# ksahlin/NGSpeciesID

Hardware: AMD Instinct MI355X
Metric: reads/sec end-to-end (cluster + spoa consensus + racon x3), 750 bp ONT (higher is better)
Workload: dtype u8 / int16 / int32 DP, 64-bit bit-vectors (f64 thresholds)

## Files before the change

### ngspeciesid_amd/csrc/k_ed_align.hip

```cpp
#include "ngsid_internal.h"
#include <algorithm>

typedef unsigned long long u64;
#define LDSP __attribute__((address_space(3)))

#define CLIP_RUN 15
template <int BMAX, bool WIN, bool CLIP = false, bool REC = false>
__global__ __launch_bounds__(64) __attribute__((amdgpu_waves_per_eu(2, 4)))
void k_ed_align(AlignJob J, ngsid_v4u* __restrict__ tb, u64 tb_per_wave , uint32_t mstride, uint32_t* __restrict__ work_ctr, int32_t* __restrict__ dist_out,
                int8_t* __restrict__ hcar ,
                int bandK , uint32_t* __restrict__ fail_list, uint32_t* __restrict__ fail_count,
                uint32_t* __restrict__ rec , uint32_t rec_stride)
{
    extern __shared__ __attribute__((aligned(16))) unsigned char smem[];
    const int lane = threadIdx.x;
    LDSP u64* planes = (LDSP u64*)smem;
    ngsid_v4u* mytb = tb + (u64)blockIdx.x * tb_per_wave;
    int8_t* myh = hcar + (u64)blockIdx.x * mstride * 64;
    const u64 npairs1 = J.npairs_dev ? (u64)*J.npairs_dev : J.npairs;
    const u64 npairs = npairs1 + (J.npairs_dev2 ? (u64)*J.npairs_dev2 : 0);
    const u64 nbundles = (npairs + 63) / 64;
    for (;;) {
        uint32_t kq = 0; if (lane == 0) kq = atomicAdd(work_ctr, 1u);
        kq = (uint32_t)__builtin_amdgcn_readfirstlane((int)kq);
        if (kq >= nbundles) break;
        const u64 pk = (u64)kq * 64 + lane;
        const bool have = pk < npairs;
        const u64 p = have ? (J.pair_list ? (pk < npairs1 ? (u64)J.pair_list[pk] : (u64)J.pair_list2[pk - npairs1]) : pk) : 0;
        const uint8_t* q = nullptr; const uint8_t* t = nullptr; int n = 0, m = 0;
        if (have) { const uint32_t qi = J.qidx[p], ti = J.tidx[p]; q = J.qseq + J.qoff[qi]; n = (int)(J.qoff[qi + 1] - J.qoff[qi]); t = J.tseq + J.toff[ti]; m = (int)(J.toff[ti + 1] - J.toff[ti]); }
        int nmax = n, mmax = m;
#pragma unroll
        for (int d = 32; d >= 1; d >>= 1) { nmax = max(nmax, __shfl_xor(nmax, d)); mmax = max(mmax, __shfl_xor(mmax, d)); }
        nmax = __builtin_amdgcn_readfirstlane(nmax); mmax = __builtin_amdgcn_readfirstlane(mmax);
        const int B = (nmax + 63) >> 6;
        const int bl = n > 0 ? (n - 1) >> 6 : 0, lastbit = n > 0 ? (n - 1) & 63 : 0;
        int score = n, best = n, bestj = 0;
        const bool band = bandK > 0 && (WIN || B <= BMAX);
        int dmin = 0, lbprev = -1, sb = 0;
        if (band) {
            dmin = have ? n - m : 0x3fffffff;
#pragma unroll
            for (int d = 32; d >= 1; d >>= 1) dmin = min(dmin, __shfl_xor(dmin, d));
            dmin = __builtin_amdgcn_readfirstlane(dmin);
        }
        if (WIN) {
            const int span = ((2 * bandK + 2 - (dmin < 0 ? dmin : 0)) >> 6) + 2;
            if (span > BMAX) {
                if (have) fail_list[atomicAdd(fail_count, 1u)] = (uint32_t)p;
                continue;
            }
        }
        int fbw = 0;
        for (int g0 = 0; g0 < B; g0 += (WIN ? B : BMAX)) {
            const int Bg = min(BMAX, B - g0);
            auto build_planes = [&](int blk, int slot) {
                u64 lo = 0, hi = 0, ok = 0;
                const int base = blk * 64;
                for (int r = 0; r < 64; ++r) {
                    const int i = base + r;
                    const int c = i < n ? ngsid_bcode(q[i]) : 4;
                    lo |= (u64)(c & 1) << r; hi |= (u64)((c >> 1) & 1) << r; ok |= (u64)(c < 4) << r;
                }
                planes[(slot * 3 + 0) * 64 + lane] = lo; planes[(slot * 3 + 1) * 64 + lane] = hi; planes[(slot * 3 + 2) * 64 + lane] = ok;
            };
            for (int b = 0; b < Bg; ++b) build_planes(g0 + b, b);
            u64 Pv[BMAX], Mv[BMAX];
#pragma unroll
            for (int b = 0; b < BMAX; ++b) { Pv[b] = ~0ull; Mv[b] = 0ull; }
            const bool more = !WIN && g0 + BMAX < B;
            u64 TPlo = 0, TPhi = 0, TPok = 0;
            for (int j = 0; j < mmax; ++j) {
                const int jb = j & 63;
                if (jb == 0) {
                    u64 lo = 0, hi = 0, ok = 0;
#pragma unroll 16
                    for (int c = 0; c < 64; ++c) {
                        const int jc = j + c;
                        const int cd = jc < m ? ngsid_bcode(t[jc]) : 4;
                        lo |= (u64)(cd & 1) << c; hi |= (u64)((cd >> 1) & 1) << c; ok |= (u64)(cd < 4) << c;
                    }
                    TPlo = lo; TPhi = hi; TPok = ok;
                }
                const u64 Tlo = 0ull - ((TPlo >> jb) & 1ull), Thi = 0ull - ((TPhi >> jb) & 1ull), Tok = 0ull - ((TPok >> jb) & 1ull);
                int fb = 0, lb = Bg - 1;
                if (band) {
                    const int lo_row = j + dmin - bandK - 1;
                    fb = lo_row > 0 ? (lo_row >> 6) : 0; lb = min(B - 1, (j + 1 + bandK) >> 6);
                    if (lb > lbprev) {
                        if (n > 0 && bl > lbprev && bl <= lb) score = sb + 64 * (bl - 1 - lbprev) + lastbit + 1;
                        sb += 64 * (lb - lbprev);
                    }
                }
                if (WIN) {
                    while (fb > fbw) {
#pragma unroll
                        for (int b = 0; b + 1 < BMAX; ++b) { Pv[b] = Pv[b + 1]; Mv[b] = Mv[b + 1]; }
                        Pv[BMAX - 1] = ~0ull; Mv[BMAX - 1] = 0ull;
                        ++fbw;
                        const int nb = fbw + BMAX - 1;
                        if (nb < B) build_planes(nb, nb % BMAX);
                    }
                }
                unsigned hp, hm;
                if (g0) { const int h0 = (int)myh[(u64)j * 64 + lane]; hp = h0 > 0; hm = h0 < 0; }
                else { hp = fb > 0 ? 1u : 0u; hm = 0u; }
                ngsid_v4u* col = mytb + ((u64)j * 64 + lane);
                const int slot0 = WIN ? fbw % BMAX : 0;
                const bool inm = j < m;
#pragma unroll
                for (int b = 0; b < BMAX; ++b) {
                    const int blk = WIN ? fbw + b : g0 + b;
                    if (WIN ? blk <= lb : (b >= fb && b <= lb)) {
                        const int ps = WIN ? (slot0 + b >= BMAX ? slot0 + b - BMAX : slot0 + b) : b;
                        const u64 lo = planes[(ps * 3 + 0) * 64 + lane], hi = planes[(ps * 3 + 1) * 64 + lane], ok = planes[(ps * 3 + 2) * 64 + lane];
                        const u64 Eq = ~((lo ^ Tlo) | (hi ^ Thi)) & ok & Tok;
                        const u64 pv = Pv[b], mv = Mv[b];
                        const u64 Xv = Eq | mv;
                        const u64 Eqh = Eq | (u64)hm;
                        const u64 Xh = (((Eqh & pv) + pv) ^ pv) | Eqh;
                        u64 Ph = mv | ~(Xh | pv), Mh = pv & Xh;
                        const u64 diag = Eq | (Ph & ~(pv | mv)) | (~(Ph | Mh) & pv);
                        if (blk == bl && inm) {
                            score += (int)((Ph >> lastbit) & 1) - (int)((Mh >> lastbit) & 1);
                            if (score < best) { best = score; bestj = j + 1; }
                        }
                        const unsigned php = (unsigned)(Ph >> 63), phm = (unsigned)(Mh >> 63);
                        Ph = (Ph << 1) | (u64)hp; Mh = (Mh << 1) | (u64)hm;
                        const u64 npv = Mh | ~(Xv | Ph);
                        Pv[b] = npv; Mv[b] = Ph & Xv;
                        ngsid_v4u w; w.x = (unsigned)diag; w.y = (unsigned)(diag >> 32); w.z = (unsigned)npv; w.w = (unsigned)(npv >> 32);
#if defined(ED_EXP_STORE_EVERY)
                        if ((j % ED_EXP_STORE_EVERY) == 0)
#endif
                        col[(u64)(WIN ? b : blk) * mstride * 64] = w;
                        hp = php; hm = phm;
                    }
                }
                if (more) myh[(u64)j * 64 + lane] = (int8_t)((int)hp - (int)hm);
                if (band) { sb += (int)hp - (int)hm; lbprev = lb; }
            }
            if (more) { asm volatile("s_waitcnt vmcnt(0)" ::: "memory"); __builtin_amdgcn_wave_barrier(); }
        }
        asm volatile("s_waitcnt vmcnt(0)" ::: "memory");
        __builtin_amdgcn_wave_barrier();
        bool ok = true;
        if (band && have && best > bandK) { ok = false; fail_list[atomicAdd(fail_count, 1u)] = (uint32_t)p; }
        int i = ok ? n : 0, j = bestj;
        int q_end = -1, t_end = -1, q_beg = -1, t_beg = -1;
        int32_t* bpp = (J.bp && have) ? J.bp + p * (u64)J.bp_windows * 4 : nullptr;
        if (bpp) for (int x = 0; x < J.bp_windows * 4; ++x) bpp[x] = -1;
        const int W = J.window > 0 ? J.window : 0x7fffffff;
        int cw = -1, w_qf = 0, w_ql = 0, w_tf = 0, w_tl = 0;
        int c_run = 0, c_x0q = -1, c_x0t = -1; bool c_started = false;
        uint32_t r_acc = 0; int r_w = -1;
        uint32_t* myrec = (REC && have) ? rec + p * (u64)rec_stride : nullptr;
        auto rec_put = [&](int ti, uint32_t nib) { const int w_ = ti >> 3; if (w_ != r_w) { if (r_w >= 0) myrec[r_w] = r_acc; r_acc = 0; r_w = w_; } r_acc |= nib << ((ti & 7) * 4); };
        int wsn = j > 0 ? (j - 1) / W : 0, ws = wsn * W;
        auto tb_blk = [&](int ii, int col0) { int tb_ = (ii - 1) >> 6; if (WIN) { const int lo_row = col0 + dmin - bandK - 1; tb_ -= lo_row > 0 ? (lo_row >> 6) : 0; } return tb_; };
        auto tb_load = [&](int tb_, int col0) { return __builtin_nontemporal_load(mytb + (((u64)tb_ * mstride + (u64)col0) * 64 + lane)); };
        int jj = i > 0 ? j : 0;
#if defined(ED_EXP_NO_TB)
        jj = 0;
#endif
#pragma unroll
        for (int d = 32; d >= 1; d >>= 1) jj = max(jj, __shfl_xor(jj, d));
        jj = __builtin_amdgcn_readfirstlane(jj);
        ngsid_v4u wn; wn.x = wn.y = wn.z = wn.w = 0; int wn_blk = -0x7fffffff;
        if (i > 0 && j == jj && jj >= 1) { wn_blk = tb_blk(i, jj - 1); wn = tb_load(wn_blk, jj - 1); }
        for (; jj >= 1; --jj) {
            if (!__ballot(i > 0 && j > 0)) break;
            const bool on = i > 0 && j == jj;
            ngsid_v4u w = wn; int wb = wn_blk;
            wn_blk = -0x7fffffff;
            if (jj >= 2) {
                int gi = 0;
                if (on && i > 1) gi = i - 1;
                else if (i > 0 && j == jj - 1) gi = i;
                if (gi > 0) { wn_blk = tb_blk(gi, jj - 2); wn = tb_load(wn_blk, jj - 2); }
            }
            if (on) {
                { const int nb = tb_blk(i, jj - 1); if (nb != wb) { w = tb_load(nb, jj - 1); wb = nb; } }
                uint32_t r_ins = 0;
                for (;;) {
                    const int bit = (i - 1) & 63;
                    const u64 dv = ((u64)w.y << 32) | w.x, uv = ((u64)w.w << 32) | w.z;
                    const bool diag = (dv >> bit) & 1, up = (uv >> bit) & 1;
                    if (diag) {
                        const int qi0 = i - 1, ti0 = j - 1;
                        auto record = [&](int qi, int ti) {
                            if (q_end < 0) { q_end = qi; t_end = ti; }
                            q_beg = qi; t_beg = ti;
                            if (bpp) {
                                while (ti < ws) { ws -= W; --wsn; }
                                const int wn_ = wsn;
                                if (wn_ != cw) { if (cw >= 0 && cw < J.bp_windows) { bpp[cw * 4 + 0] = w_qf; bpp[cw * 4 + 1] = w_ql; bpp[cw * 4 + 2] = w_tf; bpp[cw * 4 + 3] = w_tl; } cw = wn_; w_ql = qi; w_tl = ti; }
                                w_qf = qi; w_tf = ti;
                            }
                        };
                        if constexpr (CLIP) {
                            const uint8_t cq = q[qi0] & 0xDF, ct = t[ti0] & 0xDF;
                            const bool eq = cq == ct && (cq == 'A' || cq == 'C' || cq == 'G' || cq == 'T');
                            c_run = eq ? c_run + 1 : 0;
                            if (!c_started) {
                                if (c_run >= CLIP_RUN) {
                                    c_started = true;
                                    for (int d = CLIP_RUN - 1; d >= 0; --d) record(qi0 + d, ti0 + d);
                                    c_x0q = qi0; c_x0t = ti0;
                                }
                            } else {
                                record(qi0, ti0);
                                if (c_run >= CLIP_RUN) { c_x0q = qi0; c_x0t = ti0; }
                            }
                        } else record(qi0, ti0);
                        if constexpr (REC) {
                            const int cq = ngsid_bcode(q[qi0]), ct = ngsid_bcode(t[ti0]);
                            rec_put(ti0, (cq < 4 ? (cq == ct ? (uint32_t)NGSID_REC_EQ : (uint32_t)NGSID_REC_SUB + cq) : (uint32_t)NGSID_REC_OTHER) | r_ins);
                        }
                        --i; --j; break;
                    }
                    if constexpr (CLIP) c_run = 0;
                    if (!up) { if constexpr (REC) rec_put(j - 1, (uint32_t)NGSID_REC_DEL | r_ins); --j; break; }
                    --i;
                    if constexpr (REC) r_ins = NGSID_REC_INS;
                    if (i == 0) break;
                    { const int nb = tb_blk(i, jj - 1); if (nb != wb) { w = tb_load(nb, jj - 1); wb = nb; } }
                }
            }
        }
        i = 0;
        if constexpr (REC) { if (r_w >= 0) myrec[r_w] = r_acc; }
        if (bpp && ok && cw >= 0 && cw < J.bp_windows) { bpp[cw * 4 + 0] = w_qf; bpp[cw * 4 + 1] = w_ql; bpp[cw * 4 + 2] = w_tf; bpp[cw * 4 + 3] = w_tl; }
        if constexpr (CLIP) {
            if (have && ok && c_started) {
                q_beg = c_x0q; t_beg = c_x0t;
                if (bpp) { const int w0 = c_x0t / W; for (int x = 0; x < w0 && x < J.bp_windows; ++x) { bpp[x * 4 + 0] = -1; bpp[x * 4 + 1] = -1; bpp[x * 4 + 2] = -1; bpp[x * 4 + 3] = -1; }
                           if (w0 < J.bp_windows) { bpp[w0 * 4 + 0] = c_x0q; bpp[w0 * 4 + 2] = c_x0t; } }
            }
        }
        if (have && ok) {
            if (dist_out) dist_out[p] = best;
            if (J.span) { J.span[p * 4 + 0] = q_beg; J.span[p * 4 + 1] = q_end; J.span[p * 4 + 2] = t_beg; J.span[p * 4 + 3] = t_end; }
        }
        __builtin_amdgcn_wave_barrier();
    }
}

static int32_t ed_reserve(ngsid_ctx* ctx, u64& want, u64 per_wave)
{
    for (;;) {
        if (ctx->ed_tb.n >= want * per_wave) return NGSID_OK;
        hipError_t e = ctx->ed_tb.reserve(want * per_wave);
        if (e == hipSuccess) return NGSID_OK;
        (void)hipGetLastError();
        if (e != hipErrorOutOfMemory || want <= 64) HIPCHK(ctx, e);
        want = std::max<u64>(64, want / 2);
    }
}

struct EdRec { uint32_t* p = nullptr; uint32_t stride = 0; };
template <int BMAX, bool WIN = false, bool CLIP = false, bool REC = false>
static int32_t launch_ed(ngsid_ctx* ctx, const AlignJob& job, uint32_t max_qlen, uint32_t max_tlen, int32_t* dist_out, uint32_t ctr_slot = 14, int bandK = 0, uint32_t fail_slot = 15, uint32_t* fail_list = nullptr, EdRec rec = EdRec())
{
    const u64 nbundles = (job.npairs + 63) / 64;
    const uint32_t mstride = (max_tlen + 63u) & ~63u;
    const u64 nblocks = WIN ? (u64)BMAX : std::max<u64>(1, ((u64)max_qlen + 63) / 64);
    const u64 per_wave = nblocks * mstride * 64;
    const size_t lds = (size_t)BMAX * 3 * 64 * 8 + (size_t)ngsid_opt(ctx, "ed_lds_pad_kb", 0) * 1024;
    int occ = 0;
    HIPCHK(ctx, hipOccupancyMaxActiveBlocksPerMultiprocessor(&occ, k_ed_align<BMAX, WIN, CLIP, REC>, 64, lds));
    if (occ < 1) occ = 1;
    u64 want = std::min<u64>(nbundles, (u64)occ * ctx->n_cu);
    const u64 by_mem = std::max<u64>(1, std::min<size_t>((size_t)24 << 30, ctx->scratch_budget) / (per_wave * 16));
    want = std::max<u64>(1, std::min(want, by_mem));
    { int32_t rr = ed_reserve(ctx, want, per_wave); if (rr) return rr; }
    if (ctx->ed_h.n < want * (u64)mstride * 64) HIPCHK(ctx, ctx->ed_h.reserve(want * (u64)mstride * 64));
    if (ctx->aln_ctr.n < 16) HIPCHK(ctx, ctx->aln_ctr.alloc(16));
    HIPCHK(ctx, hipMemsetAsync(ctx->aln_ctr.p + ctr_slot, 0, sizeof(uint32_t), ctx->stream));
    { ProfScope ps_(ctx, REC ? "k_ed_align_rec" : "k_ed_align"); hipLaunchKernelGGL((k_ed_align<BMAX, WIN, CLIP, REC>), dim3((unsigned)want), dim3(64), lds, ctx->stream, job, ctx->ed_tb.p, per_wave, mstride, ctx->aln_ctr.p + ctr_slot, dist_out, ctx->ed_h.p,
                                                            bandK, fail_list ? fail_list : ctx->ed_fail.p, ctx->aln_ctr.p + fail_slot, rec.p, rec.stride); }
    HIPCHK(ctx, hipGetLastError());
    return NGSID_OK;
}

template <bool REC>
static int32_t launch_ed_fallback(ngsid_ctx* ctx, const AlignJob& job, uint32_t max_qlen, uint32_t max_tlen, int32_t* dist_out, int retryK, EdRec rec)
{
    AlignJob j = job; j.pair_list = ctx->ed_fail.p; j.npairs_dev = ctx->aln_ctr.p + 15; j.pair_list2 = nullptr; j.npairs_dev2 = nullptr;
    if (retryK > 0) {
        HIPCHK(ctx, ctx->ed_fail2.reserve(job.npairs));
        int32_t rc = launch_ed<8, true, false, REC>(ctx, j, max_qlen, max_tlen, dist_out, 6, retryK, 7, ctx->ed_fail2.p, rec);
        if (rc) return rc;
        j.pair_list = ctx->ed_fail2.p; j.npairs_dev = ctx->aln_ctr.p + 7;
    }
    return launch_ed<16, false, false, REC>(ctx, j, max_qlen, max_tlen, dist_out, 13, 0, 15, nullptr, rec);
}

template <bool REC>
static int32_t ed_align_route(ngsid_ctx* ctx, const AlignJob& job, uint32_t max_qlen, uint32_t max_tlen, int32_t* dist_out, EdRec rec)
{
    if (job.npairs == 0) return NGSID_OK;
    if (max_qlen > NGSID_MAX_CONSENSUS_LEN || max_tlen > NGSID_MAX_CONSENSUS_LEN) NGSID_FAIL(ctx, NGSID_ERR_TOO_LONG, "sequence longer than %d in the edit-distance aligner", NGSID_MAX_CONSENSUS_LEN);
    if (job.clip) return launch_ed<16, false, true, REC>(ctx, job, max_qlen, max_tlen, dist_out, 14, 0, 15, nullptr, rec);
    int bandK = 64 + (int)(max_qlen / 32);
    const bool band_set = ngsid_opt(ctx, "ed_band", -1) >= 0;
    if (band_set) bandK = (int)ngsid_opt(ctx, "ed_band", -1);
    const bool win = max_qlen > 1024 && bandK > 0;
    bool win16 = false;
    if (win) {
        if (bandK > 150 && !band_set) { win16 = true; bandK = std::min(64 + (int)(max_qlen / 16), 400); }
        else if (bandK > 150) { win16 = true; bandK = std::min(bandK, 400); }
    }
    if (ctx->aln_ctr.n < 16) HIPCHK(ctx, ctx->aln_ctr.alloc(16));
    if (bandK > 0) HIPCHK(ctx, ctx->ed_fail.reserve(job.npairs));
    if (job.npairs >= 4096 && max_qlen > 256 && !job.pair_list && !ngsid_opt(ctx, "align_noclass", 0)) {
        int32_t rc = ngsid_partition_pairs(ctx, job); if (rc) return rc;
        const u64 n = job.npairs;
        auto cls = [&](int c, uint32_t bound) { AlignJob j = job; j.pair_list = ctx->aln_cls.p + (size_t)c * n; j.npairs_dev = ctx->aln_ctr.p + 8 + c; (void)bound; return j; };
        {
            const uint32_t mstride = (max_tlen + 63u) & ~63u; const u64 nblocks = std::max<u64>(1, ((u64)max_qlen + 63) / 64); const u64 per_wave = nblocks * mstride * 64;
            const u64 want = std::max<u64>(1, std::min<u64>((u64)8 * ctx->n_cu, std::max<u64>(1, std::min<size_t>((size_t)24 << 30, ctx->scratch_budget) / (per_wave * 16))));
            u64 w2 = want; { int32_t rr = ed_reserve(ctx, w2, per_wave); if (rr) return rr; }
            if (ctx->ed_h.n < w2 * (u64)mstride * 64) HIPCHK(ctx, ctx->ed_h.reserve(w2 * (u64)mstride * 64));
        }
        if ((rc = launch_ed<4, false, false, REC>(ctx, cls(0, 256), std::min<uint32_t>(max_qlen, 256), max_tlen, dist_out, 1, bandK, 15, nullptr, rec))) return rc;
        if (max_qlen > 256 && (rc = launch_ed<8, false, false, REC>(ctx, cls(1, 512), std::min<uint32_t>(max_qlen, 512), max_tlen, dist_out, 2, bandK, 15, nullptr, rec))) return rc;
        const bool win_all = ngsid_opt(ctx, "ed_win_all", 1) != 0;
        const bool win2 = win_all && bandK > 0 && bandK <= 150;
        if (max_qlen > 512) {
            AlignJob j2 = cls(2, 768);
            if (win2 && max_qlen > 768) { j2.pair_list2 = ctx->aln_cls.p + (size_t)3 * n; j2.npairs_dev2 = ctx->aln_ctr.p + 8 + 3; }
            const bool win6 = win2 && bandK <= 100 && ngsid_opt(ctx, "ed_win6", 1) != 0;
            if ((rc = win6 ? launch_ed<6, true, false, REC>(ctx, j2, std::min<uint32_t>(max_qlen, 896), max_tlen, dist_out, 3, bandK, 15, nullptr, rec)
                    : win2 ? launch_ed<8, true, false, REC>(ctx, j2, std::min<uint32_t>(max_qlen, 896), max_tlen, dist_out, 3, bandK, 15, nullptr, rec)
                           : launch_ed<12, false, false, REC>(ctx, j2, std::min<uint32_t>(max_qlen, 768), max_tlen, dist_out, 3, bandK, 15, nullptr, rec))) return rc;
        }
        if (max_qlen > 768 && !win2 && (rc = launch_ed<16, false, false, REC>(ctx, cls(3, 896), std::min<uint32_t>(max_qlen, 896), max_tlen, dist_out, 4, bandK, 15, nullptr, rec))) return rc;
        if (max_qlen > 896 && (rc = win16 ? launch_ed<16, true, false, REC>(ctx, cls(4, 0), max_qlen, max_tlen, dist_out, 5, bandK, 15, nullptr, rec) : win ? launch_ed<8, true, false, REC>(ctx, cls(4, 0), max_qlen, max_tlen, dist_out, 5, bandK, 15, nullptr, rec) : launch_ed<16, false, false, REC>(ctx, cls(4, 0), max_qlen, max_tlen, dist_out, 5, bandK, 15, nullptr, rec))) return rc;
        return bandK > 0 ? launch_ed_fallback<REC>(ctx, job, max_qlen, max_tlen, dist_out, win2 ? 180 : 0, rec) : NGSID_OK;
    }
    if (bandK > 0) HIPCHK(ctx, hipMemsetAsync(ctx->aln_ctr.p + 15, 0, sizeof(uint32_t), ctx->stream));
    int32_t rc;
    if (max_qlen <= 256) rc = launch_ed<4, false, false, REC>(ctx, job, max_qlen, max_tlen, dist_out, 14, bandK, 15, nullptr, rec);
    else if (max_qlen <= 512) rc = launch_ed<8, false, false, REC>(ctx, job, max_qlen, max_tlen, dist_out, 14, bandK, 15, nullptr, rec);
    else if (max_qlen <= 768) rc = launch_ed<12, false, false, REC>(ctx, job, max_qlen, max_tlen, dist_out, 14, bandK, 15, nullptr, rec);
    else if (win16) rc = launch_ed<16, true, false, REC>(ctx, job, max_qlen, max_tlen, dist_out, 14, bandK, 15, nullptr, rec);
    else if (win) rc = launch_ed<8, true, false, REC>(ctx, job, max_qlen, max_tlen, dist_out, 14, bandK, 15, nullptr, rec);
    else rc = launch_ed<16, false, false, REC>(ctx, job, max_qlen, max_tlen, dist_out, 14, bandK, 15, nullptr, rec);
    if (rc || bandK <= 0) return rc;
    return launch_ed_fallback<REC>(ctx, job, max_qlen, max_tlen, dist_out, 0, rec);
}

int32_t ngsid_launch_ed_align(ngsid_ctx* ctx, const AlignJob& job, uint32_t max_qlen, uint32_t max_tlen, int32_t* dist_out)
{
    return ed_align_route<false>(ctx, job, max_qlen, max_tlen, dist_out, EdRec());
}

int32_t ngsid_launch_ed_align_rec(ngsid_ctx* ctx, const AlignJob& job, uint32_t max_qlen, uint32_t max_tlen, uint32_t* rec, uint32_t stride)
{
    if (!rec || !job.span || (uint64_t)stride * 8 < max_tlen) NGSID_FAIL(ctx, NGSID_ERR_ARG, "internal: path matrix of the edit-distance aligner missing or too narrow");
    EdRec r; r.p = rec; r.stride = stride;
    return ed_align_route<true>(ctx, job, max_qlen, max_tlen, nullptr, r);
}
```

Baseline: 1.462 million.

## Store band-relative shifted traceback words to cut per-column traceback writes

In the windowed banded Myers kernel, traceback diag/vertical bit-vectors are now re-aligned to the band's lower row with a funnel shift (alignbit) across adjacent blocks. This lets each column store only the minimal number of 64-bit words covering the band instead of all BMAX blocks. The traceback reader computes bit offsets relative to the band base. This cuts global-memory traceback write traffic in exchange for extra shift ALU work and more complex indexing logic.

```diff
diff --git a/ngspeciesid_amd/csrc/k_ed_align.hip b/ngspeciesid_amd/csrc/k_ed_align.hip
--- a/ngspeciesid_amd/csrc/k_ed_align.hip
+++ b/ngspeciesid_amd/csrc/k_ed_align.hip
@@ -5,6 +5,12 @@
 #define LDSP __attribute__((address_space(3)))
 
 #define CLIP_RUN 15
+__device__ __forceinline__ u64 ed_funnel(u64 lo, u64 hi, int sh)
+{
+    const bool up = sh >= 32;
+    const unsigned d0 = up ? (unsigned)(lo >> 32) : (unsigned)lo, d1 = up ? (unsigned)hi : (unsigned)(lo >> 32), d2 = up ? (unsigned)(hi >> 32) : (unsigned)hi;
+    return ((u64)__builtin_amdgcn_alignbit(d2, d1, (unsigned)sh & 31u) << 32) | (u64)__builtin_amdgcn_alignbit(d1, d0, (unsigned)sh & 31u);
+}
 template <int BMAX, bool WIN, bool CLIP = false, bool REC = false>
 __global__ __launch_bounds__(64) __attribute__((amdgpu_waves_per_eu(2, 4)))
 void k_ed_align(AlignJob J, ngsid_v4u* __restrict__ tb, u64 tb_per_wave , uint32_t mstride, uint32_t* __restrict__ work_ctr, int32_t* __restrict__ dist_out,
@@ -44,12 +50,15 @@
             for (int d = 32; d >= 1; d >>= 1) dmin = min(dmin, __shfl_xor(dmin, d));
             dmin = __builtin_amdgcn_readfirstlane(dmin);
         }
+        int relw = 0;
         if (WIN) {
             const int span = ((2 * bandK + 2 - (dmin < 0 ? dmin : 0)) >> 6) + 2;
             if (span > BMAX) {
                 if (have) fail_list[atomicAdd(fail_count, 1u)] = (uint32_t)p;
                 continue;
             }
+            const int nw = (2 * bandK + 3 - (dmin < 0 ? dmin : 0) + 63) >> 6;
+            if (band && nw < min(span, B)) relw = nw;
         }
         int fbw = 0;
         for (int g0 = 0; g0 < B; g0 += (WIN ? B : BMAX)) {
@@ -83,10 +92,11 @@
                     TPlo = lo; TPhi = hi; TPok = ok;
                 }
                 const u64 Tlo = 0ull - ((TPlo >> jb) & 1ull), Thi = 0ull - ((TPhi >> jb) & 1ull), Tok = 0ull - ((TPok >> jb) & 1ull);
-                int fb = 0, lb = Bg - 1;
+                int fb = 0, lb = Bg - 1, rsh = 0;
                 if (band) {
                     const int lo_row = j + dmin - bandK - 1;
                     fb = lo_row > 0 ? (lo_row >> 6) : 0; lb = min(B - 1, (j + 1 + bandK) >> 6);
+                    if (WIN && lo_row > 0) rsh = lo_row & 63;
                     if (lb > lbprev) {
                         if (n > 0 && bl > lbprev && bl <= lb) score = sb + 64 * (bl - 1 - lbprev) + lastbit + 1;
                         sb += 64 * (lb - lbprev);
@@ -108,9 +118,11 @@
                 ngsid_v4u* col = mytb + ((u64)j * 64 + lane);
                 const int slot0 = WIN ? fbw % BMAX : 0;
                 const bool inm = j < m;
+                u64 pdiag = 0, pnpv = 0;
 #pragma unroll
                 for (int b = 0; b < BMAX; ++b) {
                     const int blk = WIN ? fbw + b : g0 + b;
+                    u64 cdiag = 0, cnpv = 0;
                     if (WIN ? blk <= lb : (b >= fb && b <= lb)) {
                         const int ps = WIN ? (slot0 + b >= BMAX ? slot0 + b - BMAX : slot0 + b) : b;
                         const u64 lo = planes[(ps * 3 + 0) * 64 + lane], hi = planes[(ps * 3 + 1) * 64 + lane], ok = planes[(ps * 3 + 2) * 64 + lane];
@@ -130,11 +142,25 @@
                         const u64 npv = Mh | ~(Xv | Ph);
                         Pv[b] = npv; Mv[b] = Ph & Xv;
                         ngsid_v4u w; w.x = (unsigned)diag; w.y = (unsigned)(diag >> 32); w.z = (unsigned)npv; w.w = (unsigned)(npv >> 32);
+                        if (!WIN || !relw) {
 #if defined(ED_EXP_STORE_EVERY)
-                        if ((j % ED_EXP_STORE_EVERY) == 0)
+                            if ((j % ED_EXP_STORE_EVERY) == 0)
 #endif
-                        col[(u64)(WIN ? b : blk) * mstride * 64] = w;
+                            col[(u64)(WIN ? b : blk) * mstride * 64] = w;
+                        }
+                        cdiag = diag; cnpv = npv;
                         hp = php; hm = phm;
+                    }
+                    if (WIN) {
+                        if (relw && b >= 1 && b <= relw && blk - 1 <= lb) {
+                            const u64 rd = ed_funnel(pdiag, cdiag, rsh), rn = ed_funnel(pnpv, cnpv, rsh);
+                            ngsid_v4u w; w.x = (unsigned)rd; w.y = (unsigned)(rd >> 32); w.z = (unsigned)rn; w.w = (unsigned)(rn >> 32);
+#if defined(ED_EXP_STORE_EVERY)
+                            if ((j % ED_EXP_STORE_EVERY) == 0)
+#endif
+                            col[(u64)(b - 1) * mstride * 64] = w;
+                        }
+                        pdiag = cdiag; pnpv = cnpv;
                     }
                 }
                 if (more) myh[(u64)j * 64 + lane] = (int8_t)((int)hp - (int)hm);
@@ -157,7 +183,8 @@
         uint32_t* myrec = (REC && have) ? rec + p * (u64)rec_stride : nullptr;
         auto rec_put = [&](int ti, uint32_t nib) { const int w_ = ti >> 3; if (w_ != r_w) { if (r_w >= 0) myrec[r_w] = r_acc; r_acc = 0; r_w = w_; } r_acc |= nib << ((ti & 7) * 4); };
         int wsn = j > 0 ? (j - 1) / W : 0, ws = wsn * W;
-        auto tb_blk = [&](int ii, int col0) { int tb_ = (ii - 1) >> 6; if (WIN) { const int lo_row = col0 + dmin - bandK - 1; tb_ -= lo_row > 0 ? (lo_row >> 6) : 0; } return tb_; };
+        auto tb_base = [&](int col0) { if (!WIN) return 0; const int lo_row = col0 + dmin - bandK - 1; const int r0 = lo_row > 0 ? lo_row : 0; return relw ? r0 : (r0 & ~63); };
+        auto tb_blk = [&](int ii, int col0) { return (ii - 1 - tb_base(col0)) >> 6; };
         auto tb_load = [&](int tb_, int col0) { return __builtin_nontemporal_load(mytb + (((u64)tb_ * mstride + (u64)col0) * 64 + lane)); };
         int jj = i > 0 ? j : 0;
 #if defined(ED_EXP_NO_TB)
@@ -182,8 +209,9 @@
             if (on) {
                 { const int nb = tb_blk(i, jj - 1); if (nb != wb) { w = tb_load(nb, jj - 1); wb = nb; } }
                 uint32_t r_ins = 0;
+                const int rb = tb_base(jj - 1);
                 for (;;) {
-                    const int bit = (i - 1) & 63;
+                    const int bit = (i - 1 - rb) & 63;
                     const u64 dv = ((u64)w.y << 32) | w.x, uv = ((u64)w.w << 32) | w.z;
                     const bool diag = (dv >> bit) & 1, up = (uv >> bit) & 1;
                     if (diag) {
```

Result: no change. 1.470 million, median of 6 (+0.6%).
